# zhibaishouheilab/HealthiVert-GAN

Measured on NVIDIA B200. Metric: slices/sec two-stage gen fwd (256x256), higher is better.
Workload: dtype bf16

## Files before the change

### healthivert-gan_b200/csrc/ctx_attn_tc.cu

```cuda
#include <cuda_bf16.h>
#include "hv_common.cuh"
#include "kernels.h"
#include "conv_tc.cuh"

namespace hv {

int gemm_tc_nt(const __nv_bfloat16* A, const __nv_bfloat16* B, void* C, const float* colscale, int M, int N, int K, int batch,
               long long strideA, long long strideB, int out_bf16, cudaStream_t st);
int ca_mask_launch(const float* mask, float* mm, int n, int side, int mh, int mw, int per_sample, cudaStream_t st);
int ca_offsets_flow_launch(const int32_t* argmax, int32_t* offsets, float* flow, int n, int side, int up, int* scratch, cudaStream_t st);

constexpr int CA_C = 64, CA_H = 64, CA_SIDE = 32, CA_L = 1024, CA_KP = 576, CA_KR = 1024;

__global__ void __launch_bounds__(256) ca_tc_patches_kernel(TcBuf f, __nv_bfloat16* __restrict__ P, float* __restrict__ inv_norm) {
  pdl_prologue();
  const int lane = threadIdx.x & 31, gw = blockIdx.x * (blockDim.x >> 5) + (threadIdx.x >> 5);
  const int n = gw / CA_L, l = gw - n * CA_L;
  if (n >= f.n) return;
  const int lh = l >> 5, lw = l & 31;
  uint4* dst = reinterpret_cast<uint4*>(P + ((size_t)n * CA_L + l) * CA_KP);
  float ss = 0.f;
  for (int i = lane; i < 72; i += 32) {
    const int t = i >> 3, ch = i & 7, ky = t / 3, kx = t - ky * 3;
    const int y = lh + ky - 1, x = lw + kx - 1;
    uint4 v = make_uint4(0, 0, 0, 0);
    if (y >= 0 && y < CA_SIDE && x >= 0 && x < CA_SIDE)
      v = *reinterpret_cast<const uint4*>(f.ptr + f.chunk_base(n, ch) + f.pos(2 * y, 2 * x) * 8);
    dst[i] = v;
    const __nv_bfloat162* h = reinterpret_cast<const __nv_bfloat162*>(&v);
#pragma unroll
    for (int j = 0; j < 4; ++j) { const float2 q = __bfloat1622float2(h[j]); ss = fmaf(q.x, q.x, ss); ss = fmaf(q.y, q.y, ss); }
  }
  ss = warp_sum(ss);
  if (lane == 0) inv_norm[(size_t)n * CA_L + l] = 1.f / fmaxf(sqrtf(ss), 1e-4f);
}

__global__ void __launch_bounds__(256) ca_tc_raw_kernel(TcBuf f, __nv_bfloat16* __restrict__ Rt) {
  pdl_prologue();
  const int i = blockIdx.x * blockDim.x + threadIdx.x;
  const int g = i & 3, bh = (i >> 2) & 31, t = (i >> 7) & 15, ch = (i >> 11) & 7, n = i >> 14;
  if (n >= f.n) return;
  const int ky = t >> 2, kx = t & 3;
  const int y = 2 * bh - 1 + ky;
  __nv_bfloat16 v[8][8];
#pragma unroll
  for (int j = 0; j < 8; ++j) {
    const int x = 2 * (8 * g + j) - 1 + kx;
    uint4 raw = make_uint4(0, 0, 0, 0);
    if (y >= 0 && y < CA_H && x >= 0 && x < CA_H)
      raw = *reinterpret_cast<const uint4*>(f.ptr + f.chunk_base(n, ch) + f.pos(y, x) * 8);
    *reinterpret_cast<uint4*>(v[j]) = raw;
  }
#pragma unroll
  for (int c = 0; c < 8; ++c) {
    __nv_bfloat16 o[8];
#pragma unroll
    for (int j = 0; j < 8; ++j) o[j] = v[j][c];
    *reinterpret_cast<uint4*>(Rt + ((size_t)n * CA_KR + (size_t)(ch * 8 + c) * 16 + t) * CA_L + bh * CA_SIDE + 8 * g) =
        *reinterpret_cast<const uint4*>(o);
  }
}

__device__ __forceinline__ int ca_cm(int i) { return ((i & 31) << 5) | (i >> 5); }

__global__ void __launch_bounds__(256) ca_tc_fuse_softmax_kernel(const float* __restrict__ T, const float* __restrict__ mm,
                                                                 int mm_stride, __nv_bfloat16* __restrict__ A,
                                                                 int32_t* __restrict__ argmax_out, float scale, int fuse) {
  pdl_prologue();
  const int lane = threadIdx.x & 31, warp = threadIdx.x >> 5;
  const int n = blockIdx.y, j = blockIdx.x * 8 + warp;
  const float* Tn = T + (size_t)n * CA_L * CA_L;
  const float* m = mm + (size_t)n * mm_stride;
  float u[32];
#pragma unroll
  for (int k = 0; k < 32; ++k) u[k] = 0.f;
  if (fuse) {
    const int cj = ca_cm(j);
#pragma unroll
    for (int cc = -1; cc <= 1; ++cc) {
      const int pj = cj + cc;
      if (pj < 0 || pj >= CA_L) continue;
      const int q = ca_cm(pj);
#pragma unroll
      for (int a = -1; a <= 1; ++a) {
        const int s = q + a;
        if (s < 0 || s >= CA_L) continue;
        const float* row = Tn + (size_t)s * CA_L;
#pragma unroll
        for (int k = 0; k < 32; ++k) {
          const int pi = ca_cm(lane + 32 * k) + cc;
          if (pi < 0 || pi >= CA_L) continue;
          const int r = ca_cm(pi) + a;
          if (r < 0 || r >= CA_L) continue;
          u[k] += __ldg(row + r);
        }
      }
    }
  } else {
#pragma unroll
    for (int k = 0; k < 32; ++k) u[k] = __ldg(Tn + (size_t)j * CA_L + lane + 32 * k);
  }
  float mk[32];
  float mx = -INFINITY;
#pragma unroll
  for (int k = 0; k < 32; ++k) {
    mk[k] = __ldg(m + lane + 32 * k);
    u[k] = u[k] * mk[k] * scale;
    mx = fmaxf(mx, u[k]);
  }
#pragma unroll
  for (int o = 16; o > 0; o >>= 1) mx = fmaxf(mx, __shfl_xor_sync(0xffffffffu, mx, o));
  float sum = 0.f;
#pragma unroll
  for (int k = 0; k < 32; ++k) { u[k] = __expf(u[k] - mx); sum += u[k]; }
  sum = warp_sum(sum);
  const float inv = 1.f / sum;
  float best = -1.f;
  int bi = 0;
  __nv_bfloat16* out = A + ((size_t)n * CA_L + j) * CA_L;
#pragma unroll
  for (int k = 0; k < 32; ++k) {
    const float a = u[k] * inv * mk[k];
    out[lane + 32 * k] = __float2bfloat16(a);
    if (a > best) { best = a; bi = lane + 32 * k; }
  }
#pragma unroll
  for (int o = 16; o > 0; o >>= 1) {
    const float ob = __shfl_xor_sync(0xffffffffu, best, o);
    const int oi = __shfl_xor_sync(0xffffffffu, bi, o);
    if (ob > best || (ob == best && oi < bi)) { best = ob; bi = oi; }
  }
  if (lane == 0) argmax_out[(size_t)n * CA_L + j] = bi;
}

__global__ void __launch_bounds__(256) ca_tc_fold_kernel(const __nv_bfloat16* __restrict__ cols, TcBuf y) {
  pdl_prologue();
  const int i = blockIdx.x * blockDim.x + threadIdx.x;
  const int ox = i & 63, oy = (i >> 6) & 63, ch = (i >> 12) & 7, n = i >> 15;
  if (n >= y.n) return;
  const __nv_bfloat16* cn = cols + (size_t)n * CA_KR * CA_L;
  float acc[8] = {0, 0, 0, 0, 0, 0, 0, 0};
#pragma unroll
  for (int a = 0; a < 2; ++a) {
    const int ky = ((oy + 1) & 1) + 2 * a, hf = (oy + 1 - ky) >> 1;
    if (oy + 1 - ky < 0 || hf >= CA_SIDE) continue;
#pragma unroll
    for (int b = 0; b < 2; ++b) {
      const int kx = ((ox + 1) & 1) + 2 * b, wf = (ox + 1 - kx) >> 1;
      if (ox + 1 - kx < 0 || wf >= CA_SIDE) continue;
      const __nv_bfloat16* src = cn + (size_t)(ch * 8 * 16 + ky * 4 + kx) * CA_L + hf * CA_SIDE + wf;
#pragma unroll
      for (int c = 0; c < 8; ++c) acc[c] += __bfloat162float(src[(size_t)c * 16 * CA_L]);
    }
  }
  uint32_t pk[4];
#pragma unroll
  for (int e = 0; e < 4; ++e) {
    __nv_bfloat162 h = __floats2bfloat162_rn(acc[2 * e] * 0.25f, acc[2 * e + 1] * 0.25f);
    pk[e] = *reinterpret_cast<uint32_t*>(&h);
  }
  *reinterpret_cast<uint4*>(y.ptr + y.chunk_base(n, ch) + y.pos(oy, ox) * 8) = make_uint4(pk[0], pk[1], pk[2], pk[3]);
}

struct CaTcWorkspace {
  __nv_bfloat16 *P, *Rt, *A, *cols;
  float *inv_norm, *mm, *T;
  int32_t* argmax;
  int* scratch;
};

static size_t ca_tc_layout(int n, char* base, CaTcWorkspace* ws) {
  size_t off = 0;
  auto take = [&](size_t bytes) { char* p = base ? base + off : nullptr; off += (bytes + 1023) & ~(size_t)1023; return p; };
  char* p;
  p = take(sizeof(__nv_bfloat16) * n * CA_L * CA_KP);  if (ws) ws->P = (__nv_bfloat16*)p;
  p = take(sizeof(__nv_bfloat16) * n * CA_KR * CA_L);  if (ws) ws->Rt = (__nv_bfloat16*)p;
  p = take(sizeof(float) * n * CA_L * CA_L);           if (ws) ws->T = (float*)p;
  p = take(sizeof(__nv_bfloat16) * n * CA_L * CA_L);   if (ws) ws->A = (__nv_bfloat16*)p;
  p = take(sizeof(__nv_bfloat16) * n * CA_KR * CA_L);  if (ws) ws->cols = (__nv_bfloat16*)p;
  p = take(sizeof(float) * n * CA_L);                  if (ws) ws->inv_norm = (float*)p;
  p = take(sizeof(float) * n * CA_L);                  if (ws) ws->mm = (float*)p;
  p = take(sizeof(int32_t) * n * CA_L);                if (ws) ws->argmax = (int32_t*)p;
  p = take(sizeof(int) * (n + 1));                     if (ws) ws->scratch = (int*)p;
  return off;
}

size_t ctx_attn_tc_workspace_bytes(int n) { return ca_tc_layout(n, nullptr, nullptr); }

int ctx_attn_fwd_tc(const TcBuf& f, const float* mask, const TcBuf& y, int32_t* offsets, float* flow, float scale, int fuse,
                    int per_sample_mask, void* workspace, cudaStream_t st, cudaStream_t st_aux, cudaEvent_t* evs) {
  HV_CHECK_ARG(f.ptr && y.ptr && mask && workspace, "ctx_attn_fwd_tc: null argument");
  HV_CHECK_ARG(f.chunks == 8 && f.h == CA_H && f.w == CA_H && !f.s2d && y.chunks == 8 && y.h == CA_H && y.w == CA_H && !y.s2d && y.n == f.n,
               "ctx_attn_fwd_tc: built for 64-channel 64x64 feature maps");
  const int n = f.n;
  const bool two = st_aux != nullptr && evs != nullptr;
  cudaStream_t sx = two ? st_aux : st;
  CaTcWorkspace ws;
  ca_tc_layout(n, (char*)workspace, &ws);
  if (two) {
    HV_CUDA(cudaEventRecord(evs[0], st));
    HV_CUDA(cudaStreamWaitEvent(sx, evs[0], 0));
  }
  HV_CUDA(launch_pdl(ca_tc_patches_kernel, dim3((n * CA_L + 7) / 8), dim3(256), 0, st, f, ws.P, ws.inv_norm));
  HV_LAUNCH_CHECK();
  int rc = ca_mask_launch(mask, ws.mm, n, CA_SIDE, 4 * CA_H, 4 * CA_H, per_sample_mask, sx);
  if (rc) return rc;
  HV_CUDA(launch_pdl(ca_tc_raw_kernel, dim3((n * 16384 + 255) / 256), dim3(256), 0, sx, f, ws.Rt));
  HV_LAUNCH_CHECK();
  if (two) HV_CUDA(cudaEventRecord(evs[1], sx));
  rc = gemm_tc_nt(ws.P, ws.P, ws.T, ws.inv_norm, CA_L, CA_L, CA_KP, n, (long long)CA_L * CA_KP, (long long)CA_L * CA_KP, 0, st);
  if (rc) return rc;
  if (two) HV_CUDA(cudaStreamWaitEvent(st, evs[1], 0));
  HV_CUDA(launch_pdl(ca_tc_fuse_softmax_kernel, dim3(CA_L / 8, n), dim3(256), 0, st, (const float*)ws.T, (const float*)ws.mm, (int)CA_L, ws.A, ws.argmax, scale, fuse));
  HV_LAUNCH_CHECK();
  if ((offsets || flow) && two) {
    HV_CUDA(cudaEventRecord(evs[2], st));
    HV_CUDA(cudaStreamWaitEvent(sx, evs[2], 0));
    rc = ca_offsets_flow_launch(ws.argmax, offsets, flow, n, CA_SIDE, 8, ws.scratch, sx);
    if (rc) return rc;
  }
  rc = gemm_tc_nt(ws.Rt, ws.A, ws.cols, nullptr, CA_KR, CA_L, CA_L, n, (long long)CA_KR * CA_L, (long long)CA_L * CA_L, 1, st);
  if (rc) return rc;
  HV_CUDA(launch_pdl(ca_tc_fold_kernel, dim3((n * 32768 + 255) / 256), dim3(256), 0, st, (const __nv_bfloat16*)ws.cols, y));
  HV_LAUNCH_CHECK();
  if ((offsets || flow) && !two) {
    rc = ca_offsets_flow_launch(ws.argmax, offsets, flow, n, CA_SIDE, 8, ws.scratch, st);
    if (rc) return rc;
  }
  return HV_OK;
}

}
```

Before: 21300.

## Stage fuse-softmax score bands in shared memory via bulk copies; vectorize fold

Adds a persistent fuse+softmax kernel that streams bands of score rows into shared memory with mbarrier-tracked bulk copies, using a ring of five buffers. The 3x3 diagonal fuse stencil then reads from shared memory instead of re-reading global memory for every output row. It can optionally split the 32 columns across two warp halves that exchange partial sums through shared memory. The col2im fold kernel is also rewritten so each thread produces 8 adjacent output pixels from vectorized loads, replacing one gather per pixel. The cost is more code complexity, about 200KB of shared memory per block that limits occupancy to one block per SM, and a legacy environment switch.

```diff
diff --git a/healthivert-gan_b200/csrc/ctx_attn_tc.cu b/healthivert-gan_b200/csrc/ctx_attn_tc.cu
--- a/healthivert-gan_b200/csrc/ctx_attn_tc.cu
+++ b/healthivert-gan_b200/csrc/ctx_attn_tc.cu
@@ -2,6 +2,7 @@
 #include "hv_common.cuh"
 #include "kernels.h"
 #include "conv_tc.cuh"
+#include "tc_ptx.cuh"
 
 namespace hv {
 
@@ -133,7 +134,196 @@
   if (lane == 0) argmax_out[(size_t)n * CA_L + j] = bi;
 }
 
+constexpr int FS_G = 8, FS_BR = FS_G + 2, FS_RS = 1032, FS_NB = 5;
+constexpr int FS_GROUPS = (CA_SIDE / FS_G) * CA_SIDE;
+constexpr size_t fs_smem(int split) { return sizeof(float) * (FS_NB * FS_BR * FS_RS + (split > 1 ? FS_G * 16 * 32 : 0)) + sizeof(uint64_t) * FS_NB; }
+
+template <int K0, int NK>
+__device__ __forceinline__ void ca_fuse_staged(float* u, const float* const* bands, int j, int jr, int lane) {
+  const int cj = ca_cm(j);
+#pragma unroll
+  for (int cc = -1; cc <= 1; ++cc) {
+    const int pj = cj + cc;
+    if (pj < 0 || pj >= CA_L) continue;
+    const int q = ca_cm(pj);
+#pragma unroll
+    for (int a = -1; a <= 1; ++a) {
+      if (q + a < 0 || q + a >= CA_L) continue;
+      const float* row = bands[cc + 1] + (jr + a) * FS_RS;
+#pragma unroll
+      for (int kk = 0; kk < NK; ++kk) {
+        const int k = K0 + kk;
+        if (k + cc < 0) {
+          const float v = row[991 + a];
+          u[kk] += lane > 0 ? v : 0.f;
+        } else if (k + cc >= CA_SIDE) {
+          const float v = row[1 + a];
+          u[kk] += lane < CA_SIDE - 1 ? v : 0.f;
+        } else {
+          u[kk] += row[CA_SIDE * (k + cc) + a];
+        }
+      }
+    }
+  }
+}
+
+
+template <int SPLIT>
+__global__ void __launch_bounds__(FS_G * 32 * SPLIT, 1) ca_tc_fuse_softmax_staged_kernel(const float* __restrict__ T, const float* __restrict__ mm,
+                                                                                  int mm_stride, __nv_bfloat16* __restrict__ A,
+                                                                                  int32_t* __restrict__ argmax_out, float scale, int ngroups) {
+  extern __shared__ __align__(128) float fs_band[];
+  float* xch = fs_band + FS_NB * FS_BR * FS_RS;
+  uint64_t* bar = reinterpret_cast<uint64_t*>(xch + (SPLIT > 1 ? FS_G * 16 * 32 : 0));
+  const int lane = threadIdx.x & 31, row = (threadIdx.x >> 5) % FS_G, half = (threadIdx.x >> 5) / FS_G;
+  const int g0 = (int)((long long)blockIdx.x * ngroups / gridDim.x), g1 = (int)((long long)(blockIdx.x + 1) * ngroups / gridDim.x);
+  const int s0 = g0 / CA_SIDE, s_last = (g1 - 1) / CA_SIDE;
+  const int nentries = (g1 - g0) + 2 * (s_last - s0 + 1);
+  for (int i = threadIdx.x; i < FS_NB * FS_BR; i += blockDim.x) { fs_band[i * FS_RS + 3] = 0.f; fs_band[i * FS_RS + 4 + CA_L] = 0.f; }
+  if (threadIdx.x == 0) {
+    for (int b = 0; b < FS_NB; ++b) mbar_init(smem_u32(bar + b), 1);
+    fence_barrier_init();
+  }
+  __syncthreads();
+  pdl_prologue();
+  int issued = 0, ps = s0, rb = g0 % CA_SIDE - 1;
+  auto issue_until = [&](int end) {
+    end = min(end, nentries);
+    for (; issued < end; ++issued) {
+      const int slot = issued % FS_NB, n = ps / (CA_SIDE / FS_G), c0 = (ps % (CA_SIDE / FS_G)) * FS_G;
+      const int base = rb < 0 ? 991 + c0 - 1 : rb >= CA_SIDE ? c0 : CA_SIDE * rb + c0 - 1;
+      const int lo = max(base, 0), hi = min(base + FS_BR, CA_L);
+      const uint32_t b = smem_u32(bar + slot);
+      mbar_expect_tx(b, (uint32_t)((hi - lo) * CA_L * sizeof(float)));
+      for (int row = lo; row < hi; ++row)
+        bulk_load(smem_u32(fs_band + (slot * FS_BR + row - base) * FS_RS + 4), T + ((size_t)n * CA_L + row) * CA_L,
+                  CA_L * sizeof(float), b);
+      const int rend = ps == s_last ? (g1 - 1) % CA_SIDE : CA_SIDE - 1;
+      if (++rb > rend + 1) { ++ps; rb = -1; }
+    }
+  };
+  const bool producer = threadIdx.x == blockDim.x - 32;
+  if (producer) issue_until(FS_NB);
+  for (int g = g0; g < g1; ++g) {
+    const int s = g / CA_SIDE, r = g % CA_SIDE, n = s / (CA_SIDE / FS_G), c0 = (s % (CA_SIDE / FS_G)) * FS_G;
+    const int e0 = (g - g0) + 2 * (s - s0);
+#pragma unroll
+    for (int e = 0; e < 3; ++e) mbar_wait(smem_u32(bar + (e0 + e) % FS_NB), ((e0 + e) / FS_NB) & 1);
+    const int c = c0 + row, j = CA_SIDE * r + c;
+    const float* m = mm + (size_t)n * mm_stride;
+    const float* bands[3];
+#pragma unroll
+    for (int cc = -1; cc <= 1; ++cc) bands[cc + 1] = fs_band + ((e0 + 1 + cc) % FS_NB) * FS_BR * FS_RS + 4 + lane;
+    float u[32];
+#pragma unroll
+    for (int k = 0; k < 32; ++k) u[k] = 0.f;
+    if (SPLIT == 1) {
+      ca_fuse_staged<0, 32>(u, bands, j, c - c0 + 1, lane);
+    } else {
+      if (half == 0) {
+        ca_fuse_staged<0, 16>(u, bands, j, c - c0 + 1, lane);
+      } else {
+        ca_fuse_staged<16, 16>(u, bands, j, c - c0 + 1, lane);
+#pragma unroll
+        for (int kk = 0; kk < 16; ++kk) xch[(row * 16 + kk) * 32 + lane] = u[kk];
+      }
+      __syncthreads();
+      if (half == 0) {
+#pragma unroll
+        for (int kk = 0; kk < 16; ++kk) u[16 + kk] = xch[(row * 16 + kk) * 32 + lane];
+      }
+    }
+    if (half == 0) {
+    float mk[32];
+    float mx = -INFINITY;
+#pragma unroll
+    for (int k = 0; k < 32; ++k) {
+      mk[k] = __ldg(m + lane + 32 * k);
+      u[k] = u[k] * mk[k] * scale;
+      mx = fmaxf(mx, u[k]);
+    }
+#pragma unroll
+    for (int o = 16; o > 0; o >>= 1) mx = fmaxf(mx, __shfl_xor_sync(0xffffffffu, mx, o));
+    float sum = 0.f;
+#pragma unroll
+    for (int k = 0; k < 32; ++k) { u[k] = __expf(u[k] - mx); sum += u[k]; }
+    sum = warp_sum(sum);
+    const float inv = 1.f / sum;
+    float best = -1.f;
+    int bi = 0;
+    __nv_bfloat16* out = A + ((size_t)n * CA_L + j) * CA_L;
+#pragma unroll
+    for (int k = 0; k < 32; ++k) {
+      const float a = u[k] * inv * mk[k];
+      out[lane + 32 * k] = __float2bfloat16(a);
+      if (a > best) { best = a; bi = lane + 32 * k; }
+    }
+#pragma unroll
+    for (int o = 16; o > 0; o >>= 1) {
+      const float ob = __shfl_xor_sync(0xffffffffu, best, o);
+      const int oi = __shfl_xor_sync(0xffffffffu, bi, o);
+      if (ob > best || (ob == best && oi < bi)) { best = ob; bi = oi; }
+    }
+    if (lane == 0) argmax_out[(size_t)n * CA_L + j] = bi;
+    }
+    __syncthreads();
+    if (producer) issue_until((g + 1 < g1 ? e0 + 1 + ((g + 1) % CA_SIDE == 0 ? 2 : 0) : nentries) + FS_NB);
+  }
+}
+
 __global__ void __launch_bounds__(256) ca_tc_fold_kernel(const __nv_bfloat16* __restrict__ cols, TcBuf y) {
+  pdl_prologue();
+  const int i = blockIdx.x * blockDim.x + threadIdx.x;
+  const int g = i & 7, oy = (i >> 3) & 63, ch = (i >> 9) & 7, n = i >> 12;
+  if (n >= y.n) return;
+  const __nv_bfloat16* cn = cols + (size_t)n * CA_KR * CA_L;
+  float acc[8][8];
+#pragma unroll
+  for (int x = 0; x < 8; ++x)
+#pragma unroll
+    for (int c = 0; c < 8; ++c) acc[x][c] = 0.f;
+#pragma unroll
+  for (int a = 0; a < 2; ++a) {
+    const int ky = ((oy + 1) & 1) + 2 * a, hf = (oy + 1 - ky) >> 1;
+    if (oy + 1 - ky < 0 || hf >= CA_SIDE) continue;
+#pragma unroll
+    for (int c = 0; c < 8; ++c) {
+      const __nv_bfloat16* src = cn + (size_t)(ch * 8 * 16 + c * 16 + ky * 4) * CA_L + hf * CA_SIDE + 4 * g;
+      float w[4][6];
+#pragma unroll
+      for (int kx = 0; kx < 4; ++kx) {
+        const uint2 v = *reinterpret_cast<const uint2*>(src + kx * CA_L);
+        const float2 lo = __bfloat1622float2(*reinterpret_cast<const __nv_bfloat162*>(&v.x));
+        const float2 hi = __bfloat1622float2(*reinterpret_cast<const __nv_bfloat162*>(&v.y));
+        w[kx][1] = lo.x; w[kx][2] = lo.y; w[kx][3] = hi.x; w[kx][4] = hi.y;
+        w[kx][0] = w[kx][5] = 0.f;
+      }
+      if (g > 0) w[3][0] = __bfloat162float(src[3 * CA_L - 1]);
+      if (g < 7) w[0][5] = __bfloat162float(src[4]);
+#pragma unroll
+      for (int x = 0; x < 8; ++x) {
+#pragma unroll
+        for (int b = 0; b < 2; ++b) {
+          const int kx = ((x + 1) & 1) + 2 * b, d = (x + 1 - kx) >> 1;
+          if ((x == 0 && b == 1 && g == 0) || (x == 7 && b == 0 && g == 7)) continue;
+          acc[x][c] += w[kx][1 + d];
+        }
+      }
+    }
+  }
+#pragma unroll
+  for (int x = 0; x < 8; ++x) {
+    uint32_t pk[4];
+#pragma unroll
+    for (int e = 0; e < 4; ++e) {
+      __nv_bfloat162 h = __floats2bfloat162_rn(acc[x][2 * e] * 0.25f, acc[x][2 * e + 1] * 0.25f);
+      pk[e] = *reinterpret_cast<uint32_t*>(&h);
+    }
+    *reinterpret_cast<uint4*>(y.ptr + y.chunk_base(n, ch) + y.pos(oy, 8 * g + x) * 8) = make_uint4(pk[0], pk[1], pk[2], pk[3]);
+  }
+}
+
+__global__ void __launch_bounds__(256) ca_tc_fold_gather_kernel(const __nv_bfloat16* __restrict__ cols, TcBuf y) {
   pdl_prologue();
   const int i = blockIdx.x * blockDim.x + threadIdx.x;
   const int ox = i & 63, oy = (i >> 6) & 63, ch = (i >> 12) & 7, n = i >> 15;
@@ -187,6 +377,21 @@
 
 size_t ctx_attn_tc_workspace_bytes(int n) { return ca_tc_layout(n, nullptr, nullptr); }
 
+static bool ca_legacy() {
+  static const bool on = getenv("HV_CA_FUSE_LEGACY") && atoi(getenv("HV_CA_FUSE_LEGACY")) != 0;
+  return on;
+}
+
+static int ca_sm_count() {
+  static int sms = 0;
+  if (!sms) {
+    int dev = 0;
+    cudaGetDevice(&dev);
+    if (cudaDeviceGetAttribute(&sms, cudaDevAttrMultiProcessorCount, dev) != cudaSuccess || sms <= 0) sms = 148;
+  }
+  return sms;
+}
+
 int ctx_attn_fwd_tc(const TcBuf& f, const float* mask, const TcBuf& y, int32_t* offsets, float* flow, float scale, int fuse,
                     int per_sample_mask, void* workspace, cudaStream_t st, cudaStream_t st_aux, cudaEvent_t* evs) {
   HV_CHECK_ARG(f.ptr && y.ptr && mask && workspace, "ctx_attn_fwd_tc: null argument");
@@ -211,7 +416,24 @@
   rc = gemm_tc_nt(ws.P, ws.P, ws.T, ws.inv_norm, CA_L, CA_L, CA_KP, n, (long long)CA_L * CA_KP, (long long)CA_L * CA_KP, 0, st);
   if (rc) return rc;
   if (two) HV_CUDA(cudaStreamWaitEvent(st, evs[1], 0));
-  HV_CUDA(launch_pdl(ca_tc_fuse_softmax_kernel, dim3(CA_L / 8, n), dim3(256), 0, st, (const float*)ws.T, (const float*)ws.mm, (int)CA_L, ws.A, ws.argmax, scale, fuse));
+  if (fuse && !ca_legacy()) {
+    static const int split = getenv("HV_CA_FS_SPLIT") ? atoi(getenv("HV_CA_FS_SPLIT")) : 2;
+    static bool attr_set = false;
+    if (!attr_set) {
+      HV_CUDA(cudaFuncSetAttribute(ca_tc_fuse_softmax_staged_kernel<1>, cudaFuncAttributeMaxDynamicSharedMemorySize, (int)fs_smem(1)));
+      HV_CUDA(cudaFuncSetAttribute(ca_tc_fuse_softmax_staged_kernel<2>, cudaFuncAttributeMaxDynamicSharedMemorySize, (int)fs_smem(2)));
+      attr_set = true;
+    }
+    const int ngroups = n * FS_GROUPS;
+    if (split == 2)
+      HV_CUDA(launch_pdl(ca_tc_fuse_softmax_staged_kernel<2>, dim3(min(ngroups, ca_sm_count())), dim3(FS_G * 64), fs_smem(2), st,
+                         (const float*)ws.T, (const float*)ws.mm, (int)CA_L, ws.A, ws.argmax, scale, ngroups));
+    else
+      HV_CUDA(launch_pdl(ca_tc_fuse_softmax_staged_kernel<1>, dim3(min(ngroups, ca_sm_count())), dim3(FS_G * 32), fs_smem(1), st,
+                         (const float*)ws.T, (const float*)ws.mm, (int)CA_L, ws.A, ws.argmax, scale, ngroups));
+  } else {
+    HV_CUDA(launch_pdl(ca_tc_fuse_softmax_kernel, dim3(CA_L / 8, n), dim3(256), 0, st, (const float*)ws.T, (const float*)ws.mm, (int)CA_L, ws.A, ws.argmax, scale, fuse));
+  }
   HV_LAUNCH_CHECK();
   if ((offsets || flow) && two) {
     HV_CUDA(cudaEventRecord(evs[2], st));
@@ -221,7 +443,10 @@
   }
   rc = gemm_tc_nt(ws.Rt, ws.A, ws.cols, nullptr, CA_KR, CA_L, CA_L, n, (long long)CA_KR * CA_L, (long long)CA_L * CA_L, 1, st);
   if (rc) return rc;
-  HV_CUDA(launch_pdl(ca_tc_fold_kernel, dim3((n * 32768 + 255) / 256), dim3(256), 0, st, (const __nv_bfloat16*)ws.cols, y));
+  if (ca_legacy())
+    HV_CUDA(launch_pdl(ca_tc_fold_gather_kernel, dim3((n * 32768 + 255) / 256), dim3(256), 0, st, (const __nv_bfloat16*)ws.cols, y));
+  else
+    HV_CUDA(launch_pdl(ca_tc_fold_kernel, dim3((n * 4096 + 255) / 256), dim3(256), 0, st, (const __nv_bfloat16*)ws.cols, y));
   HV_LAUNCH_CHECK();
   if ((offsets || flow) && !two) {
     rc = ca_offsets_flow_launch(ws.argmax, offsets, flow, n, CA_SIDE, 8, ws.scratch, st);
```

Measured after the change: 20570, median of 6. 0.966x the previous value.
